# privacy-scaling-explorations/zkevm-specs

Measured on AMD Instinct MI355X. Metric: BN254 constraint-rows/sec, higher is better.
Workload: dtype u256 (BN254 Fr: 4xu64 canonical cells, u32-limb Montgomery); 1 GPU; EVM circuit, 2^18 execution steps per GPU, mixed-opcode synthetic trace (BASELINE configs[2]); RW table 816377 rows, bytecode table 43913 rows; steps_per_gpu=262144, rw_rows=816377, bytecode_rows=43913, witness_copies=3

## Files before the change

### include/zkevm_hip.h

```cpp
#ifndef ZKEVM_HIP_H
#define ZKEVM_HIP_H
#include <stdint.h>

#ifdef __cplusplus
extern "C" {
#endif

enum zk_kind {
    ZK_KIND_OK = 0,
    ZK_KIND_ASSERTION_ERROR = 1,
    ZK_KIND_CONSTRAINT_UNSAT = 2,
    ZK_KIND_LOOKUP_UNSAT = 3,
    ZK_KIND_LOOKUP_AMBIGUOUS = 4,
    ZK_KIND_WRONG_QUERY_KEY = 5,
    ZK_KIND_NOT_IMPLEMENTED = 6,
    ZK_KIND_TYPE_ERROR = 7,
    ZK_KIND_OVERFLOW_ERROR = 8,
    ZK_KIND_VALUE_ERROR = 9,
    ZK_KIND_ZERO_DIVISION = 10,
    ZK_KIND_INDEX_ERROR = 12,
    ZK_KIND_ATTRIBUTE_ERROR = 13,
    ZK_KIND_NAME_ERROR = 11,
    ZK_KIND_UNSUPPORTED = 15
};
// ... 163 lines not shown
    zk_copy_events copy_events;
    const uint64_t* exp_rows; uint64_t n_exp_rows;
    zk_sign_units tx;
    zk_exp_events exp_events;
} zk_block;
enum { ZK_BLOCK_EVM = 0, ZK_BLOCK_STATE = 1, ZK_BLOCK_BYTECODE = 2, ZK_BLOCK_TX = 3, ZK_BLOCK_COPY = 4, ZK_BLOCK_EXP = 5, ZK_BLOCK_NCIRCUITS = 6 };
int zk_block_verify(const zk_block* b, uint32_t opts, zk_result* results , double* chain_ms );

int zk_launch(zk_session* s, uint32_t* status_dev);
int zk_collect(zk_session* s, zk_result* result);
int zk_read_status(zk_session* s, uint32_t* status_host);
int zk_session_timing(zk_session* s, double* open_ms, double* span_ms);
int zk_last_timing(double* open_ms, double* pass_ms, double* span_ms);
int zk_timing_sums(double* sums_ms, uint64_t* count, int reset);
int zk_last_host_phases(double* us4);

#define ZK_DIST_ID_BYTES 128
typedef struct zk_comm zk_comm;
int zk_dist_unique_id(uint8_t* id );
int zk_dist_init(const uint8_t* id , int rank, int world, zk_comm** out);
int zk_dist_tally(zk_comm* c, const zk_result* local, uint64_t row_offset, zk_result* global);
int zk_dist_close(zk_comm* c);
int zk_session_set_stream(zk_session* s, void* hip_stream);
int zk_close(zk_session* s);

typedef struct zk_ecc_ops {
    const uint64_t* points;     uint64_t n_add;              uint64_t n_mul;
    const uint64_t* pair_pts;   const uint32_t* pair_off;    const uint64_t* pair_out;   uint64_t n_pairing;
    const uint64_t* randomness;
    uint32_t max_add, max_mul, max_pairing;
// ... 75 lines not shown
```

### zkevm_specs_amd/_lib.py

```python
import ctypes
import os

_HERE = os.path.dirname(os.path.abspath(__file__))
BACKEND = os.environ.get("ZK_BACKEND", "hip")
if BACKEND not in ("hip", "cpu"):
    raise ImportError(f"ZK_BACKEND={BACKEND!r}: expected 'hip' (default) or 'cpu'")
CPU_LIB_PATH = os.path.join(_HERE, "libzkevm_cpu.so")
LIB_PATH = CPU_LIB_PATH if BACKEND == "cpu" else (os.environ.get("ZK_HIP_LIB") or os.path.join(_HERE, "libzkevm_hip.so"))

EXPORTED_SYMBOLS = [
    "zk_init", "zk_shutdown", "zk_set_stream", "zk_session_set_stream", "zk_last_error", "zk_fr_op",
    "zk_state_open", "zk_state_set_range", "zk_set_range", "zk_state_verify", "zk_evm_open", "zk_evm_verify", "zk_evm_verify_batch", "zk_bytecode_open", "zk_bytecode_verify", "zk_exp_open", "zk_exp_verify", "zk_copy_open", "zk_copy_verify", "zk_sign_open", "zk_sign_verify",
    "zk_keccak_open", "zk_keccak_read_rows", "zk_keccak_table", "zk_state_assign_open", "zk_state_assign_read", "zk_state_assign", "zk_state_ops_from_rw_open", "zk_state_ops_from_rw_read", "zk_state_ops_from_rw", "zk_state_assign_from_rw_open", "zk_state_verify_from_rw_open", "zk_state_verify_from_rw", "zk_block_verify", "zk_ecdsa_open", "zk_ecdsa_open_batches", "zk_ecdsa_verify", "zk_bytecode_assign_open", "zk_bytecode_assign_read", "zk_bytecode_assign", "zk_pi_open", "zk_pi_verify", "zk_pi_copy_open", "zk_pi_copy_verify", "zk_copy_assign_sizes", "zk_copy_assign_open", "zk_copy_assign_read", "zk_copy_assign", "zk_launch", "zk_collect", "zk_read_status", "zk_close", "zk_session_timing", "zk_last_timing", "zk_timing_sums", "zk_last_host_phases", "zk_dist_unique_id", "zk_dist_init", "zk_dist_tally", "zk_dist_close",
    "zk_ecc_assign", "zk_ecc_verify", "zk_ecc_open", "zk_ecc_assign_open", "zk_ecc_assign_read", "zk_withdrawal_open", "zk_withdrawal_verify", "zk_withdrawal_assign",
    "zk_tx_assign_open", "zk_tx_assign_read", "zk_tx_assign",
    "zk_exp_assign_sizes", "zk_exp_assign_open", "zk_exp_assign_read", "zk_exp_assign", "zk_exp_assign_counts",
    "zk_pi_assign_sizes", "zk_pi_assign_open", "zk_pi_assign_read", "zk_pi_assign",
]

OPT_DEVICE_PTRS = 1


class ZkResult(ctypes.Structure):
    _fields_ = [
        ("fail_count", ctypes.c_uint64),
        ("first_fail_row", ctypes.c_uint64),
        ("first_fail_code", ctypes.c_uint32),
        ("launches", ctypes.c_uint32),
# ... 229 lines not shown
    lib.zk_exp_assign_counts.argtypes = [vp, ctypes.POINTER(u64), ctypes.POINTER(u64), ctypes.POINTER(u64)]
    lib.zk_exp_assign.argtypes = [ctypes.POINTER(ZkExpEvents), vp, vp, u32, ctypes.POINTER(ZkResult)]
    lib.zk_pi_assign_sizes.argtypes = [ctypes.POINTER(ZkPiInputs), u32, ctypes.POINTER(u64), ctypes.POINTER(u64), ctypes.POINTER(u64)]
    lib.zk_pi_assign_open.argtypes = [ctypes.POINTER(ZkPiInputs), ctypes.POINTER(ZkPiWire), u32, ctypes.POINTER(vp)]
    lib.zk_pi_assign_read.argtypes = [vp, ctypes.POINTER(ZkPiWire)]
    lib.zk_pi_assign.argtypes = [ctypes.POINTER(ZkPiInputs), ctypes.POINTER(ZkPiWire), u32, ctypes.POINTER(ZkResult)]
    lib.zk_launch.argtypes = [vp, vp]
    lib.zk_collect.argtypes = [vp, ctypes.POINTER(ZkResult)]
    lib.zk_read_status.argtypes = [vp, vp]
    lib.zk_close.argtypes = [vp]
    dp = ctypes.POINTER(ctypes.c_double)
    lib.zk_session_timing.argtypes = [vp, dp, dp]
    lib.zk_last_timing.argtypes = [dp, dp, dp]
    lib.zk_last_host_phases.argtypes = [dp]
    lib.zk_timing_sums.argtypes = [dp, ctypes.POINTER(ctypes.c_uint64), ctypes.c_int]
    lib.zk_dist_unique_id.argtypes = [ctypes.c_void_p]
    lib.zk_dist_init.argtypes = [ctypes.c_void_p, ctypes.c_int, ctypes.c_int, ctypes.POINTER(ctypes.c_void_p)]
    lib.zk_dist_tally.argtypes = [ctypes.c_void_p, ctypes.c_void_p, ctypes.c_uint64, ctypes.c_void_p]
    lib.zk_dist_close.argtypes = [ctypes.c_void_p]
    return lib


def check(rc, what, lib=None):
    if rc != 0:
        owner = lib if lib is not None else (_lib if _lib is not None else (_cpu_lib if _cpu_lib is not None else load()))
        msg = owner.zk_last_error().decode(errors="replace")
        if not msg and lib is None and _cpu_lib is not None and owner is not _cpu_lib:
            msg = _cpu_lib.zk_last_error().decode(errors="replace")
        err = EngineError(f"{what} failed (rc={rc}): {msg}")
        err.rc = int(rc)
# ... 22 lines not shown
```

### zkevm_specs_amd/csrc/cpu_backend.cpp

```cpp
#include <stdio.h>
#include <string.h>
#include <chrono>
#include <functional>
#include <string>
#include <vector>

#include "../../include/zkevm_hip.h"
#include "dist_tally.hpp"
#include "state_circuit.hpp"
#include "evm_circuit.hpp"
#include "host_index.hpp"
#include "row_circuits.hpp"
#include "copy_circuit.hpp"
#include "sign_circuit.hpp"
#include "keccak_table.hpp"
#include "secp256k1.hpp"
#include "pi_circuit.hpp"
#include "state_assign.hpp"
#include "bytecode_assign.hpp"
#include "state_rekey.hpp"
#include "ecc_circuit.hpp"
#include "withdrawal_circuit.hpp"
#include "tx_assign.hpp"
#include "exp_assign.hpp"
// ... 208 lines not shown
}
extern "C" int zk_dist_tally(zk_comm* c, const zk_result* local, uint64_t row_offset, zk_result* global) {
    ARG_TRY(c && local && global, "zk_dist_tally: bad arguments");
    uint64_t* mine = c->buf.data();
    uint64_t* all = mine + zkdist::TALLY_WORDS;
    zkdist::tally_pack(mine, local, row_offset);
    if (c->world == 1) memcpy(all, mine, zkdist::TALLY_WORDS * sizeof(uint64_t));
    else RCCL_TRY(zkdist::rccl().AllGather(mine, all, zkdist::TALLY_WORDS, zkdist::RCCL_UINT64, c->nccl, nullptr), "ncclAllGather");
    zkdist::tally_reduce(all, c->world, local, global);
    return 0;
}
extern "C" int zk_last_host_phases(double* us4) {
    if (us4) for (int k = 0; k < 4; k++) us4[k] = -1.0;
    return 0;
}
extern "C" int zk_timing_sums(double* sums_ms, uint64_t* count, int) {
    if (sums_ms) for (int k = 0; k < 3; k++) sums_ms[k] = -1.0;
    if (count) *count = 0;
    return 0;
}
extern "C" int zk_last_timing(double* open_ms, double* pass_ms, double* span_ms) {
    if (open_ms) *open_ms = -1.0;
    if (pass_ms) *pass_ms = -1.0;
    if (span_ms) *span_ms = -1.0;
    return 0;
}
extern "C" int zk_set_range(zk_session* s, uint64_t row_lo, uint64_t row_hi) {
    ARG_TRY(s && s->range_ok, "zk_set_range: not a row-circuit session");
    ARG_TRY((row_lo < row_hi || (s->range_may_be_empty && row_lo == row_hi)) && row_hi <= s->n, "zk_set_range: bad range");
    s->lo = row_lo;
// ... 1352 lines not shown
```

### zkevm_specs_amd/csrc/evm_circuit.hpp

```cpp
#pragma once
#include "common.hpp"
#include "evm_tables.h"
#include "keccak.hpp"
#include "secp_constants.h"
#include "bigz.hpp"

enum { S_STATE = 0, S_RWC, S_CALL_ID, S_IS_ROOT, S_IS_CREATE, S_CH_LO, S_CH_HI, S_PC, S_SP, S_GAS, S_MWS, S_REV, S_LOG, STEP_NCELLS };
enum { R_RWC = 0, R_RW, R_TAG, R_ID, R_ADDR, R_FT, R_KEY_LO, R_KEY_HI, R_VAL_LO, R_VAL_HI, R_PREV_LO, R_PREV_HI, R_AUX_LO, R_AUX_HI, RW_NCELLS };
enum { B_HASH_LO = 0, B_HASH_HI, B_TAG, B_INDEX, B_IS_CODE, B_VALUE, BYTECODE_NCELLS };
enum { TX_NCELLS = 5, BLOCK_NCELLS = 4 };
enum { CT_IS_FIRST = 0, CT_SRC_ID_LO, CT_SRC_ID_HI, CT_SRC_TAG, CT_DST_ID_LO, CT_DST_ID_HI, CT_DST_TAG, CT_SRC_ADDR,
       CT_SRC_ADDR_END, CT_DST_ADDR, CT_LENGTH, CT_RLC_ACC, CT_RWC, CT_RWC_INC, COPY_T_NCELLS };
enum { XT_IS_STEP = 0, XT_ID, XT_IS_LAST, XT_BASE0, XT_BASE1, XT_BASE2, XT_BASE3, XT_EXP_LO, XT_EXP_HI, XT_RES_LO, XT_RES_HI,
       EXP_T_NCELLS };
enum { SIG_T_NCELLS = 9, ECC_T_NCELLS = 13 };
enum { AUX_PAIR = 3, AUX_ECRECOVER = 5, AUX_ECADD = 6, AUX_ECMUL = 7, AUX_ECPAIRING = 8 };
enum { CDT_Bytecode = 1, CDT_Memory, CDT_TxCalldata, CDT_TxLog, CDT_RlcAcc };

struct EvmDyn {
    u32 rw_sparse;
    u32 codes_n;
    u64 rw_base;
    u32 codes_mask;
    u32 agg_max_txs, agg_total_txs, agg_invalid_txs, agg_bad_invalid_rows, agg_total_wds;
// ... 15 lines not shown
    u32 agg_rw_dups;
    const u64* aux;
    const u32* aux_kind;
    u32 aux_cells;
    u32 rw_dense;
    u64 rw_base;
    const u64* rw_keys;
    ZkCodeDir codes;
    unsigned long long* prof;
    u32* defer_list;
    u32* defer_count;
    const u32* perm;
    u32 n_pairs;
    u32 opts;
    u32* defer_count_twin;
};

ZK_HD void evm_args_resolve(EvmArgs& a) {
#ifdef EVM_RESOLVE_OFF
    return;
#endif
    if (a.dyn) {
        const EvmDyn d = *a.dyn;
        a.rw_dense = (a.rw.n != 0u && d.rw_sparse == 0u) ? 1u : 0u;
        a.rw_base = d.rw_base;
        a.codes.n = d.codes_n;
        a.codes.mask = d.codes_mask;
        a.agg_max_txs = d.agg_max_txs; a.agg_total_txs = d.agg_total_txs; a.agg_invalid_txs = d.agg_invalid_txs;
        a.agg_bad_invalid_rows = d.agg_bad_invalid_rows; a.agg_total_wds = d.agg_total_wds;
        a.agg_rw_dups = d.agg_rw_dups;
// ... 4409 lines not shown
```

### zkevm_specs_amd/csrc/evm_kernel.hpp

```cpp
#pragma once
#include "kernels.hpp"

#ifndef ZK_HOT_OCC
#define ZK_HOT_OCC 2
#endif
template <int G, int OCC, int BLOCK>
__global__ __launch_bounds__(BLOCK, OCC) void evm_steps_kernel(EvmArgs a, const u32* group_start, u32* status, ZkTally* tally) {
    u32 perm_t = 0;
    if (G == EVM_GROUP_ALL && a.perm) perm_t = a.perm[(u64)blockIdx.x * blockDim.x + threadIdx.x];
    if (G == EVM_GROUP_ALL && a.defer_count_twin != nullptr) {
        if (blockIdx.x == 0 && threadIdx.x == 0) *a.defer_count_twin = 0u;
        tally_clear_twin(tally);
    }
    __shared__ u64 s_dir[G == EVM_GROUP_ALL ? EVM_DIR_LDS_U64 : 1];
    const bool have_dir = G == EVM_GROUP_ALL && a.dyn != nullptr && a.codes.slots != nullptr && a.codes.entries != nullptr;
    if (have_dir) {
        for (u32 k = threadIdx.x; k < EVM_DIR_SLOT_U64; k += blockDim.x) s_dir[k] = (u64)a.codes.slots[2 * k] | ((u64)a.codes.slots[2 * k + 1] << 32);
        const u64* e = (const u64*)a.codes.entries;
        for (u32 k = threadIdx.x; k < EVM_DIR_MAX_ENTRIES * 12u; k += blockDim.x) s_dir[EVM_DIR_SLOT_U64 + k] = e[k];
    }
    evm_args_resolve(a);
    u32 lo = 0, hi = a.n_pairs;
    if (a.perm) {
        if (G == EVM_GROUP_ALL) hi = group_start[EVM_GROUP_WARM];
        else { lo = group_start[G]; hi = group_start[G + 1]; }
    }
    u64 t = (u64)lo + (u64)blockIdx.x * blockDim.x + threadIdx.x;
    const bool staged_launch = G == EVM_GROUP_ALL || (G == EVM_GROUP_WARM && BLOCK == EVM_HOT_BLOCK && a.perm != nullptr);
    __shared__ u32 s_stage[(G == EVM_GROUP_ALL || (G == EVM_GROUP_WARM && BLOCK == EVM_HOT_BLOCK)) ? EVM_STAGE_ENTRIES * EVM_STAGE_STRIDE : 1];
    if (staged_launch) {
      for (u32 vblock = blockIdx.x;; vblock += gridDim.x) {
        t = (u64)lo + (u64)vblock * blockDim.x + threadIdx.x;
        if ((u64)lo + (u64)vblock * blockDim.x >= (u64)hi) return;
        if (G != EVM_GROUP_ALL && vblock != blockIdx.x) __syncthreads();
        if (G != EVM_GROUP_ALL) perm_t = t < (u64)hi ? a.perm[t] : 0u;
        if (G == EVM_GROUP_ALL && EV_PROF_ON(a)) {
            a.prof[EV_PROF_WAVE * 8 + 5] = __builtin_readcyclecounter();
            a.prof[EV_PROF_WAVE * 8 + 6] = __builtin_amdgcn_s_memrealtime();
        }
        const bool dir_in_lds = have_dir && a.codes.n != 0 && a.codes.n <= EVM_DIR_MAX_ENTRIES && a.codes.mask < EVM_DIR_MAX_SLOTS;
        u32 code = 0;
        u64 idx = t;
        if (t < (u64)hi && a.perm) idx = perm_t;
        const bool mine = t < (u64)hi && idx != (u64)EVM_NO_PAIR;
        __attribute__((address_space(3))) u32* my = (__attribute__((address_space(3))) u32*)s_stage + threadIdx.x;
        const bool wide = a.step_recs ? evm_stage_steps_quad(a, (u32)idx, mine, my - (threadIdx.x & 63u))
                                      : evm_stage_steps_rows_quad(a, (u32)idx, mine, my - (threadIdx.x & 63u));
        if (dir_in_lds) __syncthreads();
// ... 9 lines not shown
                code = 0;
            } else
#else
#ifdef ZK_WARM_TWICE
            if (G == EVM_GROUP_WARM)
                code = evm_check_step<G>(a, idx, wide ? (EVM_LDS32_PTR) nullptr : (EVM_LDS32_PTR)my, (EVM_LDS_PTR) nullptr);
#endif
            code = evm_check_step<G>(a, idx, wide ? (EVM_LDS32_PTR) nullptr : (EVM_LDS32_PTR)my,
                                     dir_in_lds ? (EVM_LDS_PTR)(__attribute__((address_space(3))) u64*)s_dir : (EVM_LDS_PTR) nullptr);
#endif
            if (code == ZK_NOT_MINE) code = 0;
            else if (status) status[idx] = code;
        }
        tally_commit(tally, idx, code);
        if (G == EVM_GROUP_ALL && EV_PROF_ON(a)) a.prof[EV_PROF_WAVE * 8 + 7] = __builtin_amdgcn_s_memrealtime();
        if (G == EVM_GROUP_ALL) return;
      }
    } else {
        const u64 stride = (u64)gridDim.x * blockDim.x;
        for (; t < (u64)hi; t += stride) {
            const u64 idx = a.perm ? (u64)a.perm[t] : t;
            u32 code = idx == (u64)EVM_NO_PAIR ? (u32)ZK_NOT_MINE : evm_check_step<G>(a, idx);
            if (code == ZK_NOT_MINE) code = 0;
            else if (status) status[idx] = code;
            tally_commit(tally, idx, code);
        }
    }
}

#if defined(EVM_DEFERRED_KERNEL)
__global__ __launch_bounds__(256, 1) void evm_deferred_kernel(EvmArgs a, u32* status, ZkTally* tally) {
// ... 13 lines not shown
```

### zkevm_specs_amd/csrc/zkevm_hip.hip

```cpp
#include <hip/hip_runtime.h>
#include <hip/hip_ext.h>
#include <stdio.h>
#include <string.h>
#include <stdlib.h>
#include <chrono>
#include <string>
#include <vector>

#include <atomic>
#include <mutex>
#include <dlfcn.h>

#include "../../include/zkevm_hip.h"
#include "kernels.hpp"
#include "dist_tally.hpp"
#include "host_index.hpp"
#include "code_dir_build.hpp"

#define ZK_MAX_DEVICES 64
#define ZK_ECDSA_CHUNK_LANES (1ull << 17)
static std::mutex g_dev_mutex;
static hipStream_t g_own_stream[ZK_MAX_DEVICES] = {nullptr};
static hipStream_t g_batch_stream[ZK_MAX_DEVICES][2] = {{nullptr}};
static hipStream_t g_side_stream[ZK_MAX_DEVICES] = {nullptr};
// ... 529 lines not shown
    int evm_ranges_known = 0;
    bool evm_warm_empty = false, evm_cold_empty = false;
    u32 evm_warm_lanes = 0;
    bool deferred_pending = false;
    u32* last_status = nullptr;
    u32* d_group_start = nullptr;
    u32* d_perm = nullptr;
    hipEvent_t ev_open0 = nullptr, ev_open1 = nullptr;
    bool side_stream = false;
    hipEvent_t ev_fork = nullptr, ev_join = nullptr;
    void* d_result = nullptr;
    void* h_result = nullptr;
    u32 publish_seq = 0;
    bool publish_enqueued = false;
    u32* h_result_dev = nullptr;
    u32 early_seq = 0;
    bool tail_pending = false;
    u32 tail_cold_grid = 0;
    u32* tail_status = nullptr;
    hipEvent_t tail_e1 = nullptr;
    bool stream_drained = false;
};

static const int MAX_EVENT_PAIRS = 256;

static int session_rebind_stream(zk_session* s, hipStream_t st) {
    HIP_TRY(hipSetDevice(s->device));
    if (!st) st = g_own_stream[s->device];
    if (st == s->stream) return 0;
    HIP_TRY(hipStreamSynchronize(s->stream));
    s->stream = st;
    return 0;
}

#define ZK_ARENA_CLASSES 48
struct DevArena {
    std::mutex m;
    std::vector<void*> free_[ZK_ARENA_CLASSES];
    std::vector<hipEvent_t> events;
    std::vector<void*> pinned;
    size_t cached_bytes = 0;
};
static DevArena g_arena[ZK_MAX_DEVICES];
static size_t arena_limit() {
    static const size_t lim = [] { const char* e = getenv("ZK_ARENA_MAX_BYTES"); return e ? (size_t)strtoull(e, nullptr, 10) : ((size_t)16 << 30); }();
    return lim;
}
static bool arena_off() {
    static const bool off = [] { const char* e = getenv("ZK_NO_ARENA"); return e && e[0] == '1'; }();
    return off;
}
static int arena_class(size_t bytes) {
    int c = 8;
    while (((size_t)1 << c) < bytes) c++;
    return c;
// ... 23 lines not shown
            A.cached_bytes += (size_t)1 << cls;
            return;
        }
    }
    (void)hipFree(p);
}
#define ZK_PINNED_BYTES 256
static bool evm_poll_enabled() {
    static const bool poll = [] { const char* e = getenv("ZK_POLL_RESULT"); return !(e && e[0] == '0'); }();
    return poll;
}
static bool evm_lazy_tail_enabled() {
    static const bool lazy = [] { const char* e = getenv("ZK_LAZY_TAIL"); return !(e && e[0] == '0'); }();
    return lazy && evm_poll_enabled();
}
static int arena_pinned(int device, void** p) {
    {
        DevArena& A = g_arena[device];
        std::lock_guard<std::mutex> lock(A.m);
        if (!A.pinned.empty()) {
            *p = A.pinned.back();
            A.pinned.pop_back();
            return 0;
        }
    }
    HIP_TRY(hipHostMalloc(p, ZK_PINNED_BYTES, hipHostMallocDefault));
    return 0;
}
static int arena_event(int device, hipEvent_t* e) {
    {
        DevArena& A = g_arena[device];
        std::lock_guard<std::mutex> lock(A.m);
        if (!A.events.empty()) {
            *e = A.events.back();
            A.events.pop_back();
            return 0;
        }
    }
    HIP_TRY(hipEventCreate(e));
    return 0;
}
static void arena_release_all() {
    for (int d = 0; d < ZK_MAX_DEVICES; d++) {
        DevArena& A = g_arena[d];
        std::lock_guard<std::mutex> lock(A.m);
        bool any = !A.events.empty() || !A.pinned.empty();
        for (int c = 0; c < ZK_ARENA_CLASSES; c++) any = any || !A.free_[c].empty();
        if (!any || hipSetDevice(d) != hipSuccess) continue;
        for (int c = 0; c < ZK_ARENA_CLASSES; c++) {
            for (void* p : A.free_[c]) (void)hipFree(p);
            A.free_[c].clear();
        }
        for (hipEvent_t e : A.events) (void)hipEventDestroy(e);
        A.events.clear();
        for (void* h : A.pinned) (void)hipHostFree(h);
        A.pinned.clear();
        A.cached_bytes = 0;
    }
}

static int dev_alloc(zk_session* s, void** p, size_t bytes) {
    int cls = 0;
    int rc = arena_take(s->device, bytes, p, &cls);
    if (rc) return rc;
    s->owned.push_back(*p);
    s->owned_class.push_back(cls);
    return 0;
}
static int stage(zk_session* s, const void* src, size_t bytes, bool device_ptrs, const void** out) {
    if (bytes == 0 || !src) {
// ... 55 lines not shown
}

extern "C" int zk_close(zk_session* s) {
    if (!s) return 0;
    (void)hipSetDevice(s->device);
    if (!s->stream_drained) (void)hipStreamSynchronize(s->stream);
    for (size_t k = 0; k < s->owned.size(); k++) arena_give(s->device, s->owned[k], s->owned_class[k]);
    {
        DevArena& A = g_arena[s->device];
        std::lock_guard<std::mutex> lock(A.m);
        for (hipEvent_t e : s->ev) A.events.push_back(e);
        if (s->ev_open0) A.events.push_back(s->ev_open0);
        if (s->ev_open1) A.events.push_back(s->ev_open1);
        if (s->ev_fork) A.events.push_back(s->ev_fork);
        if (s->ev_join) A.events.push_back(s->ev_join);
        if (s->h_result) A.pinned.push_back(s->h_result);
    }
    delete s;
    return 0;
}

extern "C" int zk_state_open(const uint64_t* rows, const uint32_t* flags, uint64_t n, const uint64_t* mpt,
                             uint64_t n_mpt, uint32_t opts, zk_session** out) {
    ARG_TRY(t_device >= 0, "zk_state_open: call zk_init first");
    HIP_TRY(hipSetDevice(t_device));
    ARG_TRY(out && rows && n > 0 && n < (1ull << 32), "zk_state_open: bad arguments");
    ARG_TRY(n_mpt < (1ull << 31), "zk_state_open: MPT table too large");
    const bool dev = opts & ZK_OPT_DEVICE_PTRS;
    const bool compact = opts & ZK_OPT_STATE_COMPACT;
    zk_session* s = new zk_session();
    s->kind = SESSION_STATE;
// ... 110 lines not shown
        u32* ff = nullptr;
        if ((rc = dev_alloc(s, (void**)&ff, n_ff * sizeof(u32)))) goto fail;
        u32* cur = ff;
        for (int k = 0; k < EVM_OPEN_TABLES; k++) { small[k]->slots = cur; small[k]->mask = caps[k] - 1; cur += caps[k]; }
        E.rw.slots = cur; E.rw.mask = cap_rw - 1; cur += cap_rw;
        u32* const dir_rep = cur; cur += cap_big;
        u32* const dir_first = cur; cur += cap_big;
        u32* const small_slots = cur;
        const size_t dyn_bytes = 256, hist_bytes = EVM_N_BINS * sizeof(u32), status_bytes = (((size_t)s->n * sizeof(u32)) + 15) & ~(size_t)15;
        const size_t zero_bytes = dyn_bytes + 2 * hist_bytes + status_bytes + 3 * (size_t)cap_big * 4;
        char* zero = nullptr;
        if ((rc = dev_alloc(s, (void**)&zero, zero_bytes))) goto fail;
        EvmResultBlock* const rb = (EvmResultBlock*)zero;
        EvmDyn* dyn = &rb->dyn;
        s->d_result = rb;
        if ((rc = arena_pinned(s->device, &s->h_result))) goto fail;
        {
            void* hd = nullptr;
            if (hipHostGetDevicePointer(&hd, s->h_result, 0) == hipSuccess) s->h_result_dev = (u32*)hd;
            (void)hipGetLastError();
        }
        static_assert(sizeof(EvmResultBlock) <= 256, "the result block outgrew its slot");
        static_assert((EVM_N_BINS * sizeof(u32)) % 16 == 0, "zero region pieces are 16-byte multiples");
        s->d_hist = (u32*)(zero + dyn_bytes);
        s->d_hist2 = (u32*)(zero + dyn_bytes + hist_bytes);
        s->d_status = (u32*)(zero + dyn_bytes + 2 * hist_bytes);
        u32* const dir_last = (u32*)(zero + dyn_bytes + 2 * hist_bytes + status_bytes);
        E.dyn = dyn;
        E.defer_count = &dyn->n_deferred;
        if ((rc = dev_alloc(s, (void**)&E.defer_list, (size_t)E.n_pairs * sizeof(u32)))) goto fail;
        s->d_tally = rb->tally;
        s->tally_last = s->d_tally;
        {
            const u64 n16 = n_ff / 4 + zero_bytes / 16;
            const u32 fill_grid = (u32)(n16 / 256 < 2048 ? (n16 + 255) / 256 : 2048);
            if (arena_event(s->device, &s->ev_open0) || arena_event(s->device, &s->ev_open1)) s->ev_open0 = s->ev_open1 = nullptr;
// ... 104 lines not shown
#endif
            hipExtLaunchKernelGGL(evm_open_phase1_kernel, dim3(grid1 ? grid1 : 1u), dim3(256), 0, s->stream, nullptr, phase2 ? nullptr : s->ev_open1, 0, o);
            if (phase2)
                hipExtLaunchKernelGGL(evm_open_phase2_kernel, dim3(scatter_blocks + dir_blocks + rw_blocks), dim3(EVM_OPEN_P2_BLOCK), 0, s->stream, nullptr,
                                      s->ev_open1, 0, o, scatter_blocks, dir_blocks, generic ? 1u : 0u);
        }
        if (hipGetLastError() != hipSuccess) { rc = -2; g_err = "zk_evm_open: a build kernel failed to launch"; goto fail; }
    }
    E.opts = (t->begin_with_first_step ? 1u : 0u) | (t->end_with_last_step ? 2u : 0u);
    E.prof = nullptr;
    if (getenv("ZK_EVM_PROF")) {
        if ((rc = dev_alloc(s, (void**)&E.prof, 1024 * 4 * 8 * sizeof(unsigned long long)))) goto fail;
        if (hipMemsetAsync(E.prof, 0, 1024 * 4 * 8 * sizeof(unsigned long long), s->stream) != hipSuccess) { rc = -2; goto fail; }
    }
    E.perm = (opts & ZK_OPT_NO_STATE_SORT) ? nullptr : s->d_perm;
    *out = s;
    return 0;
fail:
    zk_close(s);
    return rc;
}

static void session_timing(zk_session* s, double pass_ms, double* open_ms, double* span_ms);
static int evm_enqueue_tail(zk_session* s);
static bool evm_publish_enqueue(zk_session* s);
extern "C" int zk_evm_verify(const zk_evm_tables* t, uint32_t opts, uint32_t* status_out, zk_result* result) {
    ARG_TRY(result, "zk_evm_verify: result is null");
    zk_session* s = nullptr;
    const auto h0 = std::chrono::steady_clock::now();
    int rc = zk_evm_open(t, opts | ZK_OPT_SINGLE_PASS, &s);
    if (rc) return rc;
    const auto h1 = std::chrono::steady_clock::now();
    const bool dev = opts & ZK_OPT_DEVICE_PTRS;
    rc = zk_launch(s, (dev && status_out) ? status_out : nullptr);
    const auto h2 = std::chrono::steady_clock::now();
    if (!rc) rc = zk_collect(s, result);
    const auto h3 = std::chrono::steady_clock::now();
    if (!rc) {
        t_timing[1] = result->kernel_ms;
        session_timing(s, result->kernel_ms, &t_timing[0], &t_timing[2]);
        for (int k = 0; k < 3; k++) t_timing_sum[k] += t_timing[k];
        t_timing_count++;
    }
    if (!rc && status_out && !dev) rc = zk_read_status(s, status_out);
    zk_close(s);
    const auto h4 = std::chrono::steady_clock::now();
    t_host_phase[0] = std::chrono::duration<double, std::micro>(h1 - h0).count();
    t_host_phase[1] = std::chrono::duration<double, std::micro>(h2 - h1).count();
// ... 1396 lines not shown
        if ((++spins & 0xfffu) == 0 && std::chrono::steady_clock::now() - t0 > std::chrono::seconds(5)) { seen = false; break; }
    }
    u32 warm_lanes = 0;
    bool run_warm = true, run_cold = true;
    if (seen) {
        warm_lanes = hw[EVM_EARLY_WORD];
        const u32 cold_lanes = hw[EVM_EARLY_WORD + 1];
        run_warm = warm_lanes != 0;
        run_cold = cold_lanes != 0;
        s->evm_ranges_known = 1;
        s->evm_warm_empty = !run_warm;
        s->evm_warm_lanes = warm_lanes;
        s->evm_cold_empty = !run_cold;
    }
    s->early_seq = 0;
    if (run_warm) zk_launch_evm_warm(s->stream, s->tail_cold_grid, warm_lanes, s->evm, s->d_group_start, s->tail_status, s->tally_last, run_cold ? nullptr : s->tail_e1);
    if (run_cold) zk_launch_evm_cold(s->stream, s->tail_cold_grid, s->evm, s->d_group_start, s->tail_status, s->tally_last, s->tail_e1);
    HIP_TRY(hipGetLastError());
    return 0;
}

extern "C" int zk_launch(zk_session* s, uint32_t* status_dev) {
    ARG_TRY(s, "zk_launch: null session");
    s->stream_drained = false;
    HIP_TRY(hipSetDevice(s->device));
    { int trc = evm_enqueue_tail(s); if (trc) return trc; }
    s->publish_enqueued = false;
    s->status_external = status_dev != nullptr;
    hipEvent_t e0 = nullptr, e1 = nullptr;
    const bool timed = s->launches < (u32)MAX_EVENT_PAIRS;
    if (timed) {
        if (s->ev.size() < 2 * (size_t)(s->launches + 1)) {
            int erc = arena_event(s->device, &e0);
            if (erc) return erc;
            s->ev.push_back(e0);
            if ((erc = arena_event(s->device, &e1))) return erc;
            s->ev.push_back(e1);
        }
        e0 = s->ev[2 * s->launches];
        e1 = s->ev[2 * s->launches + 1];
    }
    const bool twin_tally = s->kind == SESSION_STATE || s->kind == SESSION_BYTECODE || s->kind == SESSION_COPY ||
// ... 103 lines not shown
            HIP_TRY(hipEventRecord(fork, s->stream));
            HIP_TRY(hipStreamWaitEvent(side, fork, 0));
            if (run_warm)
                zk_launch_evm_warm(side, cold_grid, s->evm_ranges_known ? s->evm_warm_lanes : 0u, s->evm, s->d_group_start, status, s->tally_last, nullptr);
            if (run_cold) zk_launch_evm_cold(side, cold_grid, s->evm, s->d_group_start, status, s->tally_last, nullptr);
            HIP_TRY(hipEventRecord(s->ev_join, side));
            zk_launch_evm_hot(s->stream, grid, s->evm, s->d_group_start, status, s->tally_last, nullptr, nullptr);
            HIP_TRY(hipStreamWaitEvent(s->stream, s->ev_join, 0));
            if (status_dev && s->evm.defer_count) {
                zk_launch_evm_deferred(s->stream, s->evm, status, s->tally_last);
                s->deferred_pending = false;
            }
            break;
        }
        if (sorted && !s->evm_ranges_known && s->early_seq && !status_dev && evm_ext_events) {
            zk_launch_evm_hot(s->stream, grid, s->evm, s->d_group_start, status, s->tally_last, e0, e1);
            s->tail_pending = true;
            s->tail_cold_grid = cold_grid;
            s->tail_status = status;
            s->tail_e1 = e1;
            break;
        }
        hipEvent_t e_hot1 = (evm_ext_events && !run_warm && !run_cold) ? e1 : nullptr;
        zk_launch_evm_hot(s->stream, grid, s->evm, s->d_group_start, status, s->tally_last, evm_ext_events ? e0 : nullptr, e_hot1);
        if (run_warm)
            zk_launch_evm_warm(s->stream, cold_grid, (sorted && s->evm_ranges_known) ? s->evm_warm_lanes : 0u, s->evm, s->d_group_start, status, s->tally_last,
                               (evm_ext_events && !run_cold) ? e1 : nullptr);
        if (run_cold) zk_launch_evm_cold(s->stream, cold_grid, s->evm, s->d_group_start, status, s->tally_last, evm_ext_events ? e1 : nullptr);
        if (status_dev && s->evm.defer_count) {
            zk_launch_evm_deferred(s->stream, s->evm, status, s->tally_last);
            s->deferred_pending = false;
// ... 6 lines not shown
    s->launches++;
    return 0;
}

static int evm_finish_deferred(zk_session* s) {
    { int trc = evm_enqueue_tail(s); if (trc) return trc; }
    if (s->kind != SESSION_EVM || !s->deferred_pending || !s->evm.defer_count) return 0;
    u32 n_def = 0;
    HIP_TRY(hipMemcpyAsync(&n_def, s->evm.defer_count, 4, hipMemcpyDeviceToHost, s->stream));
    HIP_TRY(hipStreamSynchronize(s->stream));
    s->deferred_pending = false;
    if (n_def) {
        s->stream_drained = false;
        zk_launch_evm_deferred(s->stream, s->evm, s->last_status, s->tally_last);
        HIP_TRY(hipGetLastError());
    }
    return 0;
}

static bool evm_publish_enqueue(zk_session* s) {
    if (s->kind != SESSION_EVM || !s->d_result || !s->h_result || !s->h_result_dev || !evm_poll_enabled()) return false;
    u32* hw = (u32*)s->h_result;
    const u32 seq = ++s->publish_seq ? s->publish_seq : ++s->publish_seq;
    __atomic_store_n(&hw[32], 0u, __ATOMIC_RELEASE);
    hipLaunchKernelGGL(evm_publish_kernel, dim3(1), dim3(64), 0, s->stream, (const u32*)s->d_result, s->h_result_dev, seq);
    return hipGetLastError() == hipSuccess;
}

extern "C" int zk_collect(zk_session* s, zk_result* r) {
    ARG_TRY(s && r, "zk_collect: bad arguments");
    HIP_TRY(hipSetDevice(s->device));
    { int trc = evm_enqueue_tail(s); if (trc) return trc; }
    ZkTally t;
    u32 n_def = 0;
    const bool check_deferred = s->kind == SESSION_EVM && s->deferred_pending && s->evm.defer_count;
    u32 gs[EVM_N_GROUPS + 1] = {0};
    const bool read_ranges = s->kind == SESSION_EVM && s->evm.perm && !s->evm_ranges_known && s->launches > 0;
    if (s->kind == SESSION_EVM && s->d_result && s->h_result) {
        const bool poll = evm_poll_enabled();
        bool polled = false;
        if (poll) {
            static_assert(sizeof(EvmResultBlock) == 128 && ZK_PINNED_BYTES >= 4 * (EVM_EARLY_WORD + 3), "flag word behind the result block, early words behind that");
            u32* hw = (u32*)s->h_result;
            void* const hd = s->h_result_dev;
            if (hd) {
                const bool launched = s->publish_enqueued || evm_publish_enqueue(s);
                s->publish_enqueued = false;
                const u32 seq = s->publish_seq;
                if (launched) {
                    const auto t0 = std::chrono::steady_clock::now();
                    u64 spins = 0;
                    while (__atomic_load_n(&hw[32], __ATOMIC_ACQUIRE) != seq) {
                        __builtin_ia32_pause();
                        if ((++spins & 0xfffu) == 0 && std::chrono::steady_clock::now() - t0 > std::chrono::seconds(5)) break;
                    }
                    polled = __atomic_load_n(&hw[32], __ATOMIC_ACQUIRE) == seq;
                }
            }
            (void)hipGetLastError();
        }
        if (polled) {
            s->stream_drained = true;
        } else {
            HIP_TRY(hipMemcpyAsync(s->h_result, s->d_result, sizeof(EvmResultBlock), hipMemcpyDeviceToHost, s->stream));
            HIP_TRY(hipStreamSynchronize(s->stream));
        }
        const EvmResultBlock* h = (const EvmResultBlock*)s->h_result;
        n_def = s->evm_tally_idx ? h->n_deferred_twin : h->dyn.n_deferred;
        for (int k = 0; k <= EVM_N_GROUPS; k++) gs[k] = h->group_start[k];
        t = h->tally[s->tally_last - s->d_tally];
    } else {
        if (check_deferred) HIP_TRY(hipMemcpyAsync(&n_def, s->evm.defer_count, 4, hipMemcpyDeviceToHost, s->stream));
        if (read_ranges) HIP_TRY(hipMemcpyAsync(gs, s->d_group_start, sizeof gs, hipMemcpyDeviceToHost, s->stream));
        ZkTally t_asg = {0ull, ~0ull};
        if (s->fused_verify) HIP_TRY(hipMemcpyAsync(&t_asg, s->d_tally + 1, sizeof t_asg, hipMemcpyDeviceToHost, s->stream));
        HIP_TRY(hipMemcpyAsync(&t, s->tally_last, sizeof t, hipMemcpyDeviceToHost, s->stream));
        HIP_TRY(hipStreamSynchronize(s->stream));
// ... 6 lines not shown
            s->launches = 0;
            return -1;
        }
        if (s->fused_verify && s->launches > 0) s->fused_order_ready = true;
    }
    if (read_ranges) {
        s->evm_ranges_known = 1;
        s->evm_warm_empty = gs[EVM_GROUP_WARM] == gs[EVM_GROUP_WARM + 1];
        s->evm_warm_lanes = gs[EVM_GROUP_WARM + 1] - gs[EVM_GROUP_WARM];
        s->evm_cold_empty = gs[EVM_GROUP_COLD] == gs[EVM_GROUP_COLD + 1];
    }
    if (check_deferred) {
        s->deferred_pending = false;
        if (n_def) {
            s->stream_drained = false;
        zk_launch_evm_deferred(s->stream, s->evm, s->last_status, s->tally_last);
            HIP_TRY(hipGetLastError());
            HIP_TRY(hipMemcpyAsync(&t, s->tally_last, sizeof t, hipMemcpyDeviceToHost, s->stream));
            HIP_TRY(hipStreamSynchronize(s->stream));
        }
    }
    double ms = 0;
    u32 timed = s->launches < (u32)MAX_EVENT_PAIRS ? s->launches : (u32)MAX_EVENT_PAIRS;
    for (u32 k = 0; k < timed; k++) {
        float f = 0;
        hipError_t ee = hipEventElapsedTime(&f, s->ev[2 * k], s->ev[2 * k + 1]);
        if (ee == hipErrorNotReady) {
            (void)hipGetLastError();
            (void)hipEventSynchronize(s->ev[2 * k + 1]);
            ee = hipEventElapsedTime(&f, s->ev[2 * k], s->ev[2 * k + 1]);
        }
        HIP_TRY(ee);
        ms += f;
    }
    r->fail_count = t.fail_count;
    r->first_fail_row = t.first_fail == ~0ull ? UINT64_MAX : (t.first_fail >> 32);
    r->first_fail_code = t.first_fail == ~0ull ? 0u : (u32)(t.first_fail & 0xffffffffull);
    r->launches = s->launches;
    r->rows_evaluated = range_hi(s) - range_lo(s);
    r->kernel_ms = timed ? ms / timed : 0.0;
    s->launches = 0;
    return 0;
}

extern "C" int zk_read_status(zk_session* s, uint32_t* status_host) {
    ARG_TRY(s && status_host, "zk_read_status: bad arguments");
    ARG_TRY(!s->status_external, "zk_read_status: the last pass wrote its statuses to the caller's status_dev buffer, not the session's");
    HIP_TRY(hipSetDevice(s->device));
    { int drc = evm_finish_deferred(s); if (drc) return drc; }
// ... 936 lines not shown
```

Baseline: 1.612 billion rows/s.

## Publish EVM result block from last hot-kernel block directly to pinned host memory

The last block of the hot EVM kernel to finish, detected with a device-wide atomic done counter, copies the result block into pinned host memory and writes a sequence flag when the warm and cold groups are empty. This happens inside the kernel, so the separate publish kernel launch is skipped and the host can poll as soon as the hot kernel ends. It adds an atomic and a memory wait at the end of every block and a system-scope store. It also makes stream-drained tracking more complex, since timing events may still be pending after the poll returns. Launch-count statistics and an env toggle are added.

```diff
diff --git a/include/zkevm_hip.h b/include/zkevm_hip.h
--- a/include/zkevm_hip.h
+++ b/include/zkevm_hip.h
@@ -201,6 +201,7 @@
 int zk_last_timing(double* open_ms, double* pass_ms, double* span_ms);
 int zk_timing_sums(double* sums_ms, uint64_t* count, int reset);
 int zk_last_host_phases(double* us4);
+int zk_evm_publish_counts(uint64_t* counts3);
 
 #define ZK_DIST_ID_BYTES 128
 typedef struct zk_comm zk_comm;
diff --git a/zkevm_specs_amd/_lib.py b/zkevm_specs_amd/_lib.py
--- a/zkevm_specs_amd/_lib.py
+++ b/zkevm_specs_amd/_lib.py
@@ -11,7 +11,7 @@
 EXPORTED_SYMBOLS = [
     "zk_init", "zk_shutdown", "zk_set_stream", "zk_session_set_stream", "zk_last_error", "zk_fr_op",
     "zk_state_open", "zk_state_set_range", "zk_set_range", "zk_state_verify", "zk_evm_open", "zk_evm_verify", "zk_evm_verify_batch", "zk_bytecode_open", "zk_bytecode_verify", "zk_exp_open", "zk_exp_verify", "zk_copy_open", "zk_copy_verify", "zk_sign_open", "zk_sign_verify",
-    "zk_keccak_open", "zk_keccak_read_rows", "zk_keccak_table", "zk_state_assign_open", "zk_state_assign_read", "zk_state_assign", "zk_state_ops_from_rw_open", "zk_state_ops_from_rw_read", "zk_state_ops_from_rw", "zk_state_assign_from_rw_open", "zk_state_verify_from_rw_open", "zk_state_verify_from_rw", "zk_block_verify", "zk_ecdsa_open", "zk_ecdsa_open_batches", "zk_ecdsa_verify", "zk_bytecode_assign_open", "zk_bytecode_assign_read", "zk_bytecode_assign", "zk_pi_open", "zk_pi_verify", "zk_pi_copy_open", "zk_pi_copy_verify", "zk_copy_assign_sizes", "zk_copy_assign_open", "zk_copy_assign_read", "zk_copy_assign", "zk_launch", "zk_collect", "zk_read_status", "zk_close", "zk_session_timing", "zk_last_timing", "zk_timing_sums", "zk_last_host_phases", "zk_dist_unique_id", "zk_dist_init", "zk_dist_tally", "zk_dist_close",
+    "zk_keccak_open", "zk_keccak_read_rows", "zk_keccak_table", "zk_state_assign_open", "zk_state_assign_read", "zk_state_assign", "zk_state_ops_from_rw_open", "zk_state_ops_from_rw_read", "zk_state_ops_from_rw", "zk_state_assign_from_rw_open", "zk_state_verify_from_rw_open", "zk_state_verify_from_rw", "zk_block_verify", "zk_ecdsa_open", "zk_ecdsa_open_batches", "zk_ecdsa_verify", "zk_bytecode_assign_open", "zk_bytecode_assign_read", "zk_bytecode_assign", "zk_pi_open", "zk_pi_verify", "zk_pi_copy_open", "zk_pi_copy_verify", "zk_copy_assign_sizes", "zk_copy_assign_open", "zk_copy_assign_read", "zk_copy_assign", "zk_launch", "zk_collect", "zk_read_status", "zk_close", "zk_session_timing", "zk_last_timing", "zk_timing_sums", "zk_last_host_phases", "zk_evm_publish_counts", "zk_dist_unique_id", "zk_dist_init", "zk_dist_tally", "zk_dist_close",
     "zk_ecc_assign", "zk_ecc_verify", "zk_ecc_open", "zk_ecc_assign_open", "zk_ecc_assign_read", "zk_withdrawal_open", "zk_withdrawal_verify", "zk_withdrawal_assign",
     "zk_tx_assign_open", "zk_tx_assign_read", "zk_tx_assign",
     "zk_exp_assign_sizes", "zk_exp_assign_open", "zk_exp_assign_read", "zk_exp_assign", "zk_exp_assign_counts",
@@ -271,6 +271,7 @@
     lib.zk_last_timing.argtypes = [dp, dp, dp]
     lib.zk_last_host_phases.argtypes = [dp]
     lib.zk_timing_sums.argtypes = [dp, ctypes.POINTER(ctypes.c_uint64), ctypes.c_int]
+    lib.zk_evm_publish_counts.argtypes = [ctypes.POINTER(ctypes.c_uint64)]
     lib.zk_dist_unique_id.argtypes = [ctypes.c_void_p]
     lib.zk_dist_init.argtypes = [ctypes.c_void_p, ctypes.c_int, ctypes.c_int, ctypes.POINTER(ctypes.c_void_p)]
     lib.zk_dist_tally.argtypes = [ctypes.c_void_p, ctypes.c_void_p, ctypes.c_uint64, ctypes.c_void_p]
diff --git a/zkevm_specs_amd/csrc/cpu_backend.cpp b/zkevm_specs_amd/csrc/cpu_backend.cpp
--- a/zkevm_specs_amd/csrc/cpu_backend.cpp
+++ b/zkevm_specs_amd/csrc/cpu_backend.cpp
@@ -246,6 +246,10 @@
     if (us4) for (int k = 0; k < 4; k++) us4[k] = -1.0;
     return 0;
 }
+extern "C" int zk_evm_publish_counts(uint64_t* counts3) {
+    if (counts3) for (int k = 0; k < 3; k++) counts3[k] = 0;
+    return 0;
+}
 extern "C" int zk_timing_sums(double* sums_ms, uint64_t* count, int) {
     if (sums_ms) for (int k = 0; k < 3; k++) sums_ms[k] = -1.0;
     if (count) *count = 0;
diff --git a/zkevm_specs_amd/csrc/evm_circuit.hpp b/zkevm_specs_amd/csrc/evm_circuit.hpp
--- a/zkevm_specs_amd/csrc/evm_circuit.hpp
+++ b/zkevm_specs_amd/csrc/evm_circuit.hpp
@@ -53,6 +53,9 @@
     u32 n_pairs;
     u32 opts;
     u32* defer_count_twin;
+    u32* publish_host;
+    u32* done_count;
+    u32 publish_seq;
 };
 
 ZK_HD void evm_args_resolve(EvmArgs& a) {
diff --git a/zkevm_specs_amd/csrc/evm_kernel.hpp b/zkevm_specs_amd/csrc/evm_kernel.hpp
--- a/zkevm_specs_amd/csrc/evm_kernel.hpp
+++ b/zkevm_specs_amd/csrc/evm_kernel.hpp
@@ -4,6 +4,26 @@
 #ifndef ZK_HOT_OCC
 #define ZK_HOT_OCC 2
 #endif
+template <int BLOCK>
+__device__ __forceinline__ void evm_hot_block_done(const EvmArgs& a, const u32* group_start, bool worked) {
+    if (worked) {
+        asm volatile("s_waitcnt vmcnt(0)" ::: "memory");
+        if (BLOCK > 64) __syncthreads();
+    }
+    if (threadIdx.x >= 64u) return;
+    u32 prev = 0;
+    if (threadIdx.x == 0) prev = __hip_atomic_fetch_add(a.done_count, 1u, __ATOMIC_RELAXED, __HIP_MEMORY_SCOPE_AGENT);
+    prev = __builtin_amdgcn_readfirstlane(prev);
+    if (prev != gridDim.x - 1u) return;
+    if (group_start[EVM_GROUP_WARM] != group_start[EVM_GROUP_WARM + 1] || group_start[EVM_GROUP_COLD] != group_start[EVM_GROUP_COLD + 1]) return;
+    __builtin_amdgcn_fence(__ATOMIC_ACQUIRE, "agent");
+    u32* const d = (u32*)a.dyn;
+    const u32 i = threadIdx.x;
+    if (i < 32u) __hip_atomic_store(&a.publish_host[i], __hip_atomic_load(&d[i], __ATOMIC_RELAXED, __HIP_MEMORY_SCOPE_AGENT), __ATOMIC_RELAXED, __HIP_MEMORY_SCOPE_SYSTEM);
+    __builtin_amdgcn_fence(__ATOMIC_RELEASE, "");
+    asm volatile("s_waitcnt vmcnt(0)" ::: "memory");
+    if (i == 0u) __hip_atomic_store(&a.publish_host[32], a.publish_seq, __ATOMIC_RELAXED, __HIP_MEMORY_SCOPE_SYSTEM);
+}
 template <int G, int OCC, int BLOCK>
 __global__ __launch_bounds__(BLOCK, OCC) void evm_steps_kernel(EvmArgs a, const u32* group_start, u32* status, ZkTally* tally) {
     u32 perm_t = 0;
@@ -31,7 +51,10 @@
     if (staged_launch) {
       for (u32 vblock = blockIdx.x;; vblock += gridDim.x) {
         t = (u64)lo + (u64)vblock * blockDim.x + threadIdx.x;
-        if ((u64)lo + (u64)vblock * blockDim.x >= (u64)hi) return;
+        if ((u64)lo + (u64)vblock * blockDim.x >= (u64)hi) {
+            if (G == EVM_GROUP_ALL && a.publish_host != nullptr) evm_hot_block_done<BLOCK>(a, group_start, false);
+            return;
+        }
         if (G != EVM_GROUP_ALL && vblock != blockIdx.x) __syncthreads();
         if (G != EVM_GROUP_ALL) perm_t = t < (u64)hi ? a.perm[t] : 0u;
         if (G == EVM_GROUP_ALL && EV_PROF_ON(a)) {
@@ -71,7 +94,10 @@
         }
         tally_commit(tally, idx, code);
         if (G == EVM_GROUP_ALL && EV_PROF_ON(a)) a.prof[EV_PROF_WAVE * 8 + 7] = __builtin_amdgcn_s_memrealtime();
-        if (G == EVM_GROUP_ALL) return;
+        if (G == EVM_GROUP_ALL) {
+            if (a.publish_host != nullptr) evm_hot_block_done<BLOCK>(a, group_start, true);
+            return;
+        }
       }
     } else {
         const u64 stride = (u64)gridDim.x * blockDim.x;
diff --git a/zkevm_specs_amd/csrc/zkevm_hip.hip b/zkevm_specs_amd/csrc/zkevm_hip.hip
--- a/zkevm_specs_amd/csrc/zkevm_hip.hip
+++ b/zkevm_specs_amd/csrc/zkevm_hip.hip
@@ -567,6 +567,8 @@
     u32 publish_seq = 0;
     bool publish_enqueued = false;
     u32* h_result_dev = nullptr;
+    bool inkernel_allowed = false;
+    bool inkernel_armed = false;
     u32 early_seq = 0;
     bool tail_pending = false;
     u32 tail_cold_grid = 0;
@@ -591,7 +593,8 @@
     std::mutex m;
     std::vector<void*> free_[ZK_ARENA_CLASSES];
     std::vector<hipEvent_t> events;
-    std::vector<void*> pinned;
+    struct Pinned { void* host; u32* dev; };
+    std::vector<Pinned> pinned;
     size_t cached_bytes = 0;
 };
 static DevArena g_arena[ZK_MAX_DEVICES];
@@ -645,17 +648,25 @@
     static const bool lazy = [] { const char* e = getenv("ZK_LAZY_TAIL"); return !(e && e[0] == '0'); }();
     return lazy && evm_poll_enabled();
 }
-static int arena_pinned(int device, void** p) {
+static bool evm_inkernel_publish_enabled() {
+    static const bool on = [] { const char* e = getenv("ZK_INKERNEL_PUBLISH"); return !(e && e[0] == '0'); }();
+    return on && evm_lazy_tail_enabled();
+}
+static int arena_pinned(int device, void** p, u32** dev) {
     {
         DevArena& A = g_arena[device];
         std::lock_guard<std::mutex> lock(A.m);
         if (!A.pinned.empty()) {
-            *p = A.pinned.back();
+            *p = A.pinned.back().host;
+            *dev = A.pinned.back().dev;
             A.pinned.pop_back();
             return 0;
         }
     }
     HIP_TRY(hipHostMalloc(p, ZK_PINNED_BYTES, hipHostMallocDefault));
+    void* hd = nullptr;
+    *dev = hipHostGetDevicePointer(&hd, *p, 0) == hipSuccess ? (u32*)hd : nullptr;
+    (void)hipGetLastError();
     return 0;
 }
 static int arena_event(int device, hipEvent_t* e) {
@@ -684,7 +695,7 @@
         }
         for (hipEvent_t e : A.events) (void)hipEventDestroy(e);
         A.events.clear();
-        for (void* h : A.pinned) (void)hipHostFree(h);
+        for (const DevArena::Pinned& h : A.pinned) (void)hipHostFree(h.host);
         A.pinned.clear();
         A.cached_bytes = 0;
     }
@@ -770,7 +781,7 @@
         if (s->ev_open1) A.events.push_back(s->ev_open1);
         if (s->ev_fork) A.events.push_back(s->ev_fork);
         if (s->ev_join) A.events.push_back(s->ev_join);
-        if (s->h_result) A.pinned.push_back(s->h_result);
+        if (s->h_result) A.pinned.push_back({s->h_result, s->h_result_dev});
     }
     delete s;
     return 0;
@@ -911,12 +922,7 @@
         EvmResultBlock* const rb = (EvmResultBlock*)zero;
         EvmDyn* dyn = &rb->dyn;
         s->d_result = rb;
-        if ((rc = arena_pinned(s->device, &s->h_result))) goto fail;
-        {
-            void* hd = nullptr;
-            if (hipHostGetDevicePointer(&hd, s->h_result, 0) == hipSuccess) s->h_result_dev = (u32*)hd;
-            (void)hipGetLastError();
-        }
+        if ((rc = arena_pinned(s->device, &s->h_result, &s->h_result_dev))) goto fail;
         static_assert(sizeof(EvmResultBlock) <= 256, "the result block outgrew its slot");
         static_assert((EVM_N_BINS * sizeof(u32)) % 16 == 0, "zero region pieces are 16-byte multiples");
         s->d_hist = (u32*)(zero + dyn_bytes);
@@ -1051,6 +1057,8 @@
         if (hipMemsetAsync(E.prof, 0, 1024 * 4 * 8 * sizeof(unsigned long long), s->stream) != hipSuccess) { rc = -2; goto fail; }
     }
     E.perm = (opts & ZK_OPT_NO_STATE_SORT) ? nullptr : s->d_perm;
+    E.publish_host = E.done_count = nullptr;
+    E.publish_seq = 0;
     *out = s;
     return 0;
 fail:
@@ -1059,6 +1067,11 @@
 }
 
 static void session_timing(zk_session* s, double pass_ms, double* open_ms, double* span_ms);
+static std::atomic<uint64_t> g_publish_counts[3];
+extern "C" int zk_evm_publish_counts(uint64_t* counts3) {
+    if (counts3) for (int k = 0; k < 3; k++) counts3[k] = g_publish_counts[k].load(std::memory_order_relaxed);
+    return 0;
+}
 static int evm_enqueue_tail(zk_session* s);
 static bool evm_publish_enqueue(zk_session* s);
 extern "C" int zk_evm_verify(const zk_evm_tables* t, uint32_t opts, uint32_t* status_out, zk_result* result) {
@@ -1069,6 +1082,7 @@
     if (rc) return rc;
     const auto h1 = std::chrono::steady_clock::now();
     const bool dev = opts & ZK_OPT_DEVICE_PTRS;
+    s->inkernel_allowed = !status_out;
     rc = zk_launch(s, (dev && status_out) ? status_out : nullptr);
     const auto h2 = std::chrono::steady_clock::now();
     if (!rc) rc = zk_collect(s, result);
@@ -2495,6 +2509,7 @@
         s->evm_cold_empty = !run_cold;
     }
     s->early_seq = 0;
+    if (run_warm || run_cold) s->inkernel_armed = false;
     if (run_warm) zk_launch_evm_warm(s->stream, s->tail_cold_grid, warm_lanes, s->evm, s->d_group_start, s->tail_status, s->tally_last, run_cold ? nullptr : s->tail_e1);
     if (run_cold) zk_launch_evm_cold(s->stream, s->tail_cold_grid, s->evm, s->d_group_start, s->tail_status, s->tally_last, s->tail_e1);
     HIP_TRY(hipGetLastError());
@@ -2507,6 +2522,7 @@
     HIP_TRY(hipSetDevice(s->device));
     { int trc = evm_enqueue_tail(s); if (trc) return trc; }
     s->publish_enqueued = false;
+    s->inkernel_armed = false;
     s->status_external = status_dev != nullptr;
     hipEvent_t e0 = nullptr, e1 = nullptr;
     const bool timed = s->launches < (u32)MAX_EVENT_PAIRS;
@@ -2640,7 +2656,16 @@
             break;
         }
         if (sorted && !s->evm_ranges_known && s->early_seq && !status_dev && evm_ext_events) {
-            zk_launch_evm_hot(s->stream, grid, s->evm, s->d_group_start, status, s->tally_last, e0, e1);
+            EvmArgs hot = s->evm;
+            if (s->inkernel_allowed && evm_inkernel_publish_enabled() && s->h_result_dev && s->d_result) {
+                const u32 seq = ++s->publish_seq ? s->publish_seq : ++s->publish_seq;
+                __atomic_store_n(&((u32*)s->h_result)[32], 0u, __ATOMIC_RELEASE);
+                hot.publish_host = s->h_result_dev;
+                hot.publish_seq = seq;
+                hot.done_count = (u32*)((char*)s->d_result + 128);
+                s->inkernel_armed = true;
+            }
+            zk_launch_evm_hot(s->stream, grid, hot, s->d_group_start, status, s->tally_last, e0, e1);
             s->tail_pending = true;
             s->tail_cold_grid = cold_grid;
             s->tail_status = status;
@@ -2677,6 +2702,7 @@
         s->stream_drained = false;
         zk_launch_evm_deferred(s->stream, s->evm, s->last_status, s->tally_last);
         HIP_TRY(hipGetLastError());
+        g_publish_counts[2]++;
     }
     return 0;
 }
@@ -2687,6 +2713,7 @@
     const u32 seq = ++s->publish_seq ? s->publish_seq : ++s->publish_seq;
     __atomic_store_n(&hw[32], 0u, __ATOMIC_RELEASE);
     hipLaunchKernelGGL(evm_publish_kernel, dim3(1), dim3(64), 0, s->stream, (const u32*)s->d_result, s->h_result_dev, seq);
+    g_publish_counts[0]++;
     return hipGetLastError() == hipSuccess;
 }
 
@@ -2696,19 +2723,23 @@
     { int trc = evm_enqueue_tail(s); if (trc) return trc; }
     ZkTally t;
     u32 n_def = 0;
+    bool inkernel = false, inkernel_polled = false;
     const bool check_deferred = s->kind == SESSION_EVM && s->deferred_pending && s->evm.defer_count;
     u32 gs[EVM_N_GROUPS + 1] = {0};
     const bool read_ranges = s->kind == SESSION_EVM && s->evm.perm && !s->evm_ranges_known && s->launches > 0;
     if (s->kind == SESSION_EVM && s->d_result && s->h_result) {
         const bool poll = evm_poll_enabled();
         bool polled = false;
+        if (!poll) s->inkernel_armed = false;
         if (poll) {
             static_assert(sizeof(EvmResultBlock) == 128 && ZK_PINNED_BYTES >= 4 * (EVM_EARLY_WORD + 3), "flag word behind the result block, early words behind that");
             u32* hw = (u32*)s->h_result;
             void* const hd = s->h_result_dev;
             if (hd) {
-                const bool launched = s->publish_enqueued || evm_publish_enqueue(s);
+                inkernel = s->inkernel_armed;
+                const bool launched = inkernel || s->publish_enqueued || evm_publish_enqueue(s);
                 s->publish_enqueued = false;
+                s->inkernel_armed = false;
                 const u32 seq = s->publish_seq;
                 if (launched) {
                     const auto t0 = std::chrono::steady_clock::now();
@@ -2723,7 +2754,9 @@
             (void)hipGetLastError();
         }
         if (polled) {
-            s->stream_drained = true;
+            s->stream_drained = !inkernel;
+            if (inkernel) g_publish_counts[1]++;
+            inkernel_polled = inkernel;
         } else {
             HIP_TRY(hipMemcpyAsync(s->h_result, s->d_result, sizeof(EvmResultBlock), hipMemcpyDeviceToHost, s->stream));
             HIP_TRY(hipStreamSynchronize(s->stream));
@@ -2760,8 +2793,10 @@
         s->deferred_pending = false;
         if (n_def) {
             s->stream_drained = false;
-        zk_launch_evm_deferred(s->stream, s->evm, s->last_status, s->tally_last);
+            inkernel_polled = false;
+            zk_launch_evm_deferred(s->stream, s->evm, s->last_status, s->tally_last);
             HIP_TRY(hipGetLastError());
+            g_publish_counts[2]++;
             HIP_TRY(hipMemcpyAsync(&t, s->tally_last, sizeof t, hipMemcpyDeviceToHost, s->stream));
             HIP_TRY(hipStreamSynchronize(s->stream));
         }
@@ -2779,6 +2814,7 @@
         HIP_TRY(ee);
         ms += f;
     }
+    if (inkernel_polled && timed && timed == s->launches) s->stream_drained = true;
     r->fail_count = t.fail_count;
     r->first_fail_row = t.first_fail == ~0ull ? UINT64_MAX : (t.first_fail >> 32);
     r->first_fail_code = t.first_fail == ~0ull ? 0u : (u32)(t.first_fail & 0xffffffffull);
```

Result: slower. 1.523 billion rows/s (-5.5%).
